# iamycy/golf

Hardware: AMD Instinct MI355X
Metric: audio samples/sec (24 kHz) GOLF-ss synth, batch=32x2 s, 4 batches in flight (higher is better)
Workload: dtype f32

## Files before the change

golf_amd/csrc/device_common.h:

```cpp
#pragma once
#include <hip/hip_runtime.h>

namespace golf {

struct BufRow {
    __amdgpu_buffer_rsrc_t rs;
    __device__ __forceinline__ BufRow(const float* p, int T)
        : rs(__builtin_amdgcn_make_buffer_rsrc((void*)p, 0, T * 4, 0x00020000)) {}
    __device__ __forceinline__ float ld(int t) const {
        return __builtin_bit_cast(float, __builtin_amdgcn_raw_buffer_load_b32(rs, t * 4, 0, 0));
    }
    __device__ __forceinline__ void st(int t, float v) const {
        __builtin_amdgcn_raw_buffer_store_b32(__builtin_bit_cast(unsigned, v), rs, t * 4, 0, 0);
    }
};

template <int W, int ROWS = 64>
struct Tile {
    static constexpr int LD = W + 1;
    static constexpr int SIZE = ROWS * LD;
    static constexpr int ITS = ROWS * W / 64;

    __device__ static __forceinline__ void rowcol(int it, int lq, int lr, int& row, int& col) {
        const int q = (it * 64) / W, r = (it * 64) % W;
        col = r + lr;
        row = q + lq;
        if (col >= W) { col -= W; row += 1; }
        if (col >= W) { col -= W; row += 1; }
    }
    template <int DIR = 1>
    __device__ static __forceinline__ void fetch(float (&r)[ITS], const BufRow& src, int tbase, int L, int lq,
                                                 int lr) {
#pragma unroll
        for (int it = 0; it < ITS; ++it) {
            int row, col;
            rowcol(it, lq, lr, row, col);
            r[it] = src.ld(tbase + row * L + DIR * col);
        }
    }
    template <int DIR = 1>
    __device__ static __forceinline__ void store(const float (&r)[ITS], const BufRow& dst, int tbase, int L, int lq,
                                                 int lr) {
#pragma unroll
        for (int it = 0; it < ITS; ++it) {
            int row, col;
            rowcol(it, lq, lr, row, col);
            dst.st(tbase + row * L + DIR * col, r[it]);
        }
    }
    __device__ static __forceinline__ void scatter(float* lds, const float (&r)[ITS], int lq, int lr) {
#pragma unroll
        for (int it = 0; it < ITS; ++it) {
            int row, col;
            rowcol(it, lq, lr, row, col);
            lds[row * LD + col] = r[it];
        }
    }
    __device__ static __forceinline__ void gather(float (&r)[ITS], const float* lds, int lq, int lr) {
#pragma unroll
        for (int it = 0; it < ITS; ++it) {
            int row, col;
            rowcol(it, lq, lr, row, col);
            r[it] = lds[row * LD + col];
        }
    }
    __device__ static __forceinline__ void rows_load(float (&x)[W], const float* lds, int row) {
#pragma unroll
        for (int s = 0; s < W; ++s) x[s] = lds[row * LD + s];
    }
    __device__ static __forceinline__ void rows_store(float* lds, const float (&x)[W], int row) {
#pragma unroll
        for (int s = 0; s < W; ++s) lds[row * LD + s] = x[s];
    }
};

#ifndef GOLF_PRIO_LIGHT
#define GOLF_PRIO_LIGHT 1
#endif
__device__ __forceinline__ void light_wave_priority() {
#if GOLF_PRIO_LIGHT > 0
    __builtin_amdgcn_s_setprio(GOLF_PRIO_LIGHT);
#endif
}

__device__ __forceinline__ void wave_lds_fence() {
    __builtin_amdgcn_fence(__ATOMIC_RELEASE, "wavefront", "local");
    __builtin_amdgcn_wave_barrier();
    __builtin_amdgcn_fence(__ATOMIC_ACQUIRE, "wavefront", "local");
}

__device__ __forceinline__ float lane_bcast(float v, int lane) {
    return __int_as_float(__builtin_amdgcn_readlane(__float_as_int(v), lane));
}
__device__ __forceinline__ float f4get(const float4& v, int k) {
    return k == 0 ? v.x : (k == 1 ? v.y : (k == 2 ? v.z : v.w));
}


constexpr int quad_tpl(int W, int NT) {
    for (int d = 1; d <= W; ++d)
        if (W % d == 0 && 4 * d >= NT) return d;
    return W;
}
template <int CTRL>
__device__ __forceinline__ float dppf(float v) {
    return __builtin_bit_cast(float, __builtin_amdgcn_update_dpp(0, __builtin_bit_cast(int, v), CTRL, 0xF, 0xF, false));
}
#define DPP_XOR1 0xB1
#define DPP_XOR2 0x4E
#define DPP_SHR1 0x90
#define DPP_SHL1 0xF9
#define DPP_BC0  0x00


}
```

golf_amd/csrc/lpc_ss.hip:

```cpp
#include "common.h"
#include "device_common.h"
#include "lpc_p1f.h"
#include <cstdlib>

namespace golf {

struct WNT { int W, NT; };
static const WNT kTable[] = {{8, 2},   {8, 4},   {8, 6},   {16, 8},  {16, 12}, {16, 14}, {24, 8},  {24, 12},
                             {24, 16}, {24, 20}, {24, 22}, {32, 16}, {32, 22}, {32, 26}, {32, 30}, {40, 22},
                             {40, 26}, {40, 32}, {40, 38}};

#ifndef GOLF_SS_SERIAL_MIN_BATCH
#define GOLF_SS_SERIAL_MIN_BATCH 2048
#endif

bool make_ss_plan(int B, int T, int F, int M, int hop, SsPlan* p, int mode) {
    p->W = 0;
    p->NT = 0;
    p->serial = mode == GOLF_SS_SERIAL || (mode != GOLF_SS_CHUNKED && B >= GOLF_SS_SERIAL_MIN_BATCH);
    if (F >= 2) {
        for (const WNT& e : kTable) {
            if (e.NT < M || hop % e.W != 0) continue;
            if (p->W == 0 || e.NT < p->NT || (e.NT == p->NT && e.W < p->W)) { p->W = e.W; p->NT = e.NT; }
        }
    }
    if (p->W == 0) { p->total = 256; return false; }
    const int W = p->W;
    int L;
    const int target = 240;
    if (hop >= target) {
        L = W;
        for (int cand = W; cand <= 256 && cand <= hop; cand += W)
            if (hop % cand == 0) L = cand;
    } else {
        L = hop * (target / hop);
    }
    p->L = L;
    p->NC = (int)ceil_div(T, L);
    p->NP = p->NC - 1;
    p->seg = L < hop ? L : hop;
    p->NSEG = (int)ceil_div(T, p->seg);
    size_t o = 0;
    if (p->serial) {
        p->off_phi = p->off_phiT = p->off_z = p->off_E = p->off_z2 = p->off_S = p->off_zadj = p->off_lam = 0;
        p->NG = p->GS = 0;
        p->off_mt = p->off_gv = p->off_pmax = 0;
        p->off_tier = p->off_S1 = p->off_status = p->off_phi64 = p->off_fixcnt = 0;
        p->off_m64 = p->off_v64 = p->off_g64 = 0;
        p->off_mtT = p->off_L1 = p->off_wadj = p->off_dadj = 0;
        p->off_gflag = 0;
        p->off_g = o;    o = align_up(o + sizeof(float) * (size_t)B * T, 256);
        p->off_pa = o;   o = align_up(o + sizeof(float) * (size_t)B * p->NSEG * 2 * W, 256);
        p->off_pg = o;   o = align_up(o + sizeof(float) * (size_t)B * p->NSEG * 2, 256);
        p->total = o;
        return true;
    }
    p->off_phi = o;  o = align_up(o + sizeof(float) * (size_t)B * (p->NP > 0 ? p->NP : 1) * p->NT * W, 256);
    p->off_phiT = o; o = align_up(o + sizeof(float) * (size_t)B * (p->NP > 0 ? p->NP : 1) * p->NT * W, 256);
    p->off_z = o;    o = align_up(o + sizeof(float) * (size_t)B * (p->NP > 0 ? p->NP : 1) * W, 256);
    p->off_E = o;    o = align_up(o + sizeof(float) * (size_t)B * (p->NP > 0 ? p->NP : 1) * W, 256);
    p->off_z2 = o;   o = align_up(o + sizeof(float) * (size_t)B * (p->NP > 0 ? p->NP : 1) * W, 256);
    p->off_S = o;    o = align_up(o + sizeof(float) * (size_t)B * p->NC * 64, 256);
    p->off_zadj = o; o = align_up(o + sizeof(float) * (size_t)B * p->NC * W, 256);
    p->off_lam = o;  o = align_up(o + sizeof(float) * (size_t)B * p->NC * 64, 256);
    p->off_g = o;    o = align_up(o + sizeof(float) * (size_t)B * T, 256);
    p->off_pa = o;   o = align_up(o + sizeof(float) * (size_t)B * p->NSEG * 2 * W, 256);
    p->off_pg = o;   o = align_up(o + sizeof(float) * (size_t)B * p->NSEG * 2, 256);
    p->off_pmax = o; o = align_up(o + sizeof(float) * (size_t)B * (p->NP > 0 ? p->NP : 1), 256);
    p->off_tier = o; o = align_up(o + sizeof(unsigned) * ((size_t)B * 2 + 2), 256);
    p->off_status = o; o = align_up(o + sizeof(unsigned) * 8, 256);
    p->off_fixcnt = o; o = align_up(o + sizeof(unsigned) * ((size_t)B * 5 + 1), 256);
    p->NG = 0;
    p->GS = 0;
    p->off_mt = p->off_gv = o;
    if (p->NP >= 48 && p->NT <= 24) {
        p->GS = 16;
        p->NG = (int)ceil_div(p->NP, p->GS);
        p->off_mt = o;   o = align_up(o + sizeof(float) * (size_t)B * p->NG * p->NT * W, 256);
        p->off_gv = o; o = align_up(o + sizeof(float) * (size_t)B * p->NG * 32 * 2, 256);
    }
    p->off_S1 = o;   o = align_up(o + sizeof(float) * (size_t)B * p->NC * 32, 256);
    p->off_mtT = o;  o = align_up(o + sizeof(float) * (size_t)B * (p->NG > 0 ? p->NG : 1) * p->NT * W, 256);
    p->off_L1 = o;   o = align_up(o + sizeof(float) * (size_t)B * (p->NC + 1) * 32, 256);
    p->off_wadj = o; o = align_up(o + sizeof(float) * (size_t)B * (p->NG > 0 ? p->NG : 1) * 32 * 2, 256);
    p->off_dadj = o; o = align_up(o + sizeof(float) * (size_t)B * p->NC * W, 256);
    p->off_phi64 = o; o = align_up(o + sizeof(double) * (size_t)B * (p->NP > 0 ? p->NP : 1) * p->NT * W, 256);
    p->off_m64 = o;  o = align_up(o + sizeof(double) * (size_t)B * (p->NG > 0 ? p->NG : 1) * p->NT * W, 256);
    p->off_v64 = o;  o = align_up(o + sizeof(double) * (size_t)B * (p->NG > 0 ? p->NG : 1) * 32, 256);
    p->off_g64 = o;  o = align_up(o + sizeof(double) * (size_t)B * (p->NG + 1) * 32, 256);
    p->off_gflag = o; o = align_up(o + sizeof(unsigned) * (size_t)B * (p->NG + 1), 256);
    p->total = o;
    return true;
}

static float phi_guard() {
    static const float v = [] { const char* e = getenv("GOLF_SS_PHI_GUARD"); return e ? (float)atof(e) : 30.f; }();
    return v;
}
static float phi_guard2() {
    static const float v = [] { const char* e = getenv("GOLF_SS_PHI_GUARD2"); return e ? (float)atof(e) : 8.f; }();
    return v;
}
static float group_log2_guard() {
    static const float v = [] { const char* e = getenv("GOLF_SS_GROUP_LOG2"); return e ? (float)atof(e) : 96.f; }();
    return v;
}
static int hot_all_16ths() {
    static const int v = [] { const char* e = getenv("GOLF_SS_HOT_ALL_16THS"); return e ? atoi(e) : 16; }();
    return v;
}
static int hot_count() {
    static const int v = [] { const char* e = getenv("GOLF_SS_HOT_COUNT"); return e ? atoi(e) : 160; }();
    return v;
}
static float phi_guard3() {
    static const float v = [] { const char* e = getenv("GOLF_SS_PHI_GUARD3"); return e ? (float)atof(e) : 256.f; }();
    return v;
}
static bool serial_strides_ok(int64_t s0, int64_t s1) { return s0 < (1 << 24) && s1 < (1 << 24); }
constexpr unsigned kTierHot = 2u, kTierPrecise = 3u;
constexpr unsigned kScanTwoLevel = 0x2C0DE001u, kScanFlat = 0x2C0DE002u;
__device__ __forceinline__ void record_scan_kind(const unsigned* tier, int B, unsigned kind) {
    if (tier) { unsigned* w = const_cast<unsigned*>(tier); w[2 * B] = kind; w[2 * B + 1] = 0u; }
}
__device__ __forceinline__ void check_scan_kind(const unsigned* tier, int B, unsigned kind) {
    if (tier && tier[2 * B] != kind) const_cast<unsigned*>(tier)[2 * B + 1] = 1u;
}
__device__ __forceinline__ bool tier3(const unsigned* __restrict__ tier, int b) {
    return tier != nullptr && __builtin_amdgcn_readfirstlane((int)tier[2 * b]) == (int)kTierPrecise;
}

template <int W, int NT, int MODE, bool LS = false>
__device__ __forceinline__ void fwdq_body(const float* __restrict__ ex, int64_t ex_stride,
                                          const float* __restrict__ gain, const float* __restrict__ a,
                                          const float* __restrict__ S, float* __restrict__ out, int64_t y_stride, int T,
                                          int F, int M, int hop, int L, int NCQ, int NCS,
                                          const float* __restrict__ zin, float* __restrict__ xt,
                                          float* __restrict__ yt, int b, int cg, int lane,
                                          const float* lst = nullptr, float* ldl = nullptr,
                                          unsigned* __restrict__ nonfinite = nullptr) {
    constexpr int TPL = quad_tpl(W, NT);
    constexpr bool WY = MODE == 1;
    static_assert(MODE >= 0 && MODE <= 3 && (MODE != 3 || LS), "MODE 3 exists only with LDS-resident start states");
    constexpr int R = 16;
    using TL = Tile<W, R>;
    const int lq = lane / W, lr = lane % W;
    const int row = lane >> 2, r = lane & 3;
    const int c0 = cg * R;
    const int c = c0 + row;
    const bool mine = c < NCQ;
    const BufRow xrow(ex + (size_t)b * ex_stride, T);
    const BufRow yrow(WY ? out + (size_t)b * y_stride : nullptr, WY ? T : 0);
    float w[TPL];
    if (MODE >= 1 && mine) {
        if constexpr (LS) {
#pragma unroll
            for (int k = 0; k < TPL; ++k) w[TPL - 1 - k] = lst[row * 32 + r * TPL + k];
        } else {
            const float* sp = S + ((size_t)b * NCS + c) * 64 + r * TPL;
#pragma unroll
            for (int k = 0; k < TPL; ++k) w[TPL - 1 - k] = sp[k];
        }
    } else {
#pragma unroll
        for (int k = 0; k < TPL; ++k) w[k] = 0.f;
    }
    float a0[TPL], dd[TPL];
#pragma unroll
    for (int k = 0; k < TPL; ++k) { a0[k] = 0.f; dd[k] = 0.f; }
    float g0 = 0.f, dg = 0.f;
    const float inv_hop = 1.0f / (float)hop;
    int fcur = -1;
    const int nblk = L / W;
    float nx[TL::ITS];
    bool bad = false;
    TL::fetch(nx, xrow, c0 * L, L, lq, lr);
    for (int blk = 0; blk < nblk; ++blk) {
        const int tw = c0 * L + blk * W;
        if (tw >= T) break;
        TL::scatter(xt, nx, lq, lr);
        wave_lds_fence();
        float xin[W];
        TL::rows_load(xin, xt, row);
        TL::fetch(nx, xrow, tw + W, L, lq, lr);
        const int t0 = c * L + blk * W;
        const bool act = mine && t0 < T;
        float keep[W / 4];
#pragma unroll
        for (int j = 0; j < W / 4; ++j) keep[j] = 0.f;
        if (act) {
            int f = t0 / hop;
            if (f > F - 2) f = F - 2;
            if (f != fcur) {
                fcur = f;
                const float* pa0 = a + ((size_t)b * F + f) * M;
                const float* pa1 = pa0 + M;
#pragma unroll
                for (int k = 0; k < TPL; ++k) {
                    const int i = r * TPL + k;
                    const float v0 = i < M ? pa0[i] : 0.f;
                    const float v1 = i < M ? pa1[i] : 0.f;
                    a0[k] = v0;
                    dd[k] = (v1 - v0) * inv_hop;
                }
                g0 = gain[(size_t)b * F + f];
                dg = (gain[(size_t)b * F + f + 1] - g0) * inv_hop;
            }
            const float n0 = (float)(t0 - f * hop);
#pragma unroll
            for (int s = 0; s < W; ++s) {
                const float n = n0 + (float)s;
                const float x = xin[s] * fmaf(n, dg, g0);
                float cf[TPL];
#pragma unroll
                for (int k = 0; k < TPL; ++k) cf[k] = fmaf(n, dd[k], a0[k]);
                float pa = 0.f, pb = 0.f;
#pragma unroll
                for (int k = TPL - 1; k >= 1; --k) {
                    const int slot = (s - 1 - k + 4 * TPL) % TPL;
                    if (k & 1) pa = fmaf(cf[k], w[slot], pa);
                    else       pb = fmaf(cf[k], w[slot], pb);
                }
                float part = fmaf(cf[0], w[(s - 1 + TPL) % TPL], pa + pb);
                part += dppf<DPP_XOR1>(part);
                part += dppf<DPP_XOR2>(part);
                const float y = x - part;
                const float oldest = w[s % TPL];
                const float inc = dppf<DPP_SHR1>(oldest);
                w[s % TPL] = r == 0 ? y : inc;
                if (WY) keep[s >> 2] = ((s & 3) == r) ? y : keep[s >> 2];
            }
        }
        if (WY) {
#pragma unroll
            for (int j = 0; j < W / 4; ++j) yt[row * TL::LD + 4 * j + r] = keep[j];
            wave_lds_fence();
            float o[TL::ITS];
            TL::gather(o, yt, lq, lr);
            TL::store(o, yrow, tw, L, lq, lr);
#pragma unroll
            for (int it = 0; it < TL::ITS; ++it) bad = bad || !(fabsf(o[it]) <= 3.4028235e38f);
        }
        wave_lds_fence();
    }
    if (WY && nonfinite && __builtin_amdgcn_ballot_w64(bad) != 0ull && lane == 0) atomicOr(nonfinite, 1u);
    if (!WY && mine) {
        float* zp = out + ((size_t)b * NCQ + c) * W;
#pragma unroll
        for (int k = 0; k < TPL; ++k) {
            const int i = r * TPL + k;
            if (i < W) {
                float v = i < M ? w[TPL - 1 - k] : 0.f;
                if (MODE == 2) v -= S[((size_t)b * NCS + c + 1) * 64 + i];
                if constexpr (MODE == 3) {
                    v -= lst[(row + 1) * 32 + i];
                    ldl[row * 32 + i] = v;
                    if (!out) continue;
                }
                if constexpr (MODE == 0) {
                    if (ldl) ldl[row * 32 + i] = v;
                }
                zp[i] = v;
            }
        }
    }
}

template <int W, int NT, int MODE>
__global__ __launch_bounds__(64) void lpc_fwdq_kernel(const float* __restrict__ ex, int64_t ex_stride,
                                                      const float* __restrict__ gain, const float* __restrict__ a,
                                                      const float* __restrict__ S, float* __restrict__ out,
                                                      int64_t y_stride, int T, int F, int M, int hop, int L, int NCQ,
                                                      int NCS, const float* __restrict__ zin,
                                                      const unsigned* __restrict__ tier = nullptr) {
    using TL = Tile<W, 16>;
    __shared__ float xt[TL::SIZE];
    __shared__ float yt[MODE == 1 ? TL::SIZE : 1];
    if (MODE == 2 && tier3(tier, blockIdx.y)) return;
    fwdq_body<W, NT, MODE>(ex, ex_stride, gain, a, S, out, y_stride, T, F, M, hop, L, NCQ, NCS, zin, xt, yt,
                           blockIdx.y, blockIdx.x, threadIdx.x);
}

template <int CTRL>
__device__ __forceinline__ float dpp_row(float v) {
    return __builtin_bit_cast(float, __builtin_amdgcn_update_dpp(0, __builtin_bit_cast(int, v), CTRL, 0xF, 0xF, true));
}
template <int W, int NT, int LPU, bool STATE = false>
__device__ __forceinline__ void serial_fwd_unit(int unit, float* __restrict__ xt, float* __restrict__ yt,
                                                const float* __restrict__ ex, int64_t ex_stride,
                                                const float* __restrict__ gain, const float* __restrict__ a,
                                                float* __restrict__ y, int64_t y_stride, int B, int T, int F, int M,
                                                int hop, float* state = nullptr) {
    static_assert(LPU == 4 || LPU == 8, "a quad or half a DPP row per utterance");
    constexpr int ROWS = 64 / LPU;
    constexpr int TPL = LPU == 4 ? quad_tpl(W, NT) : (NT + LPU - 1) / LPU;
    static_assert(W % LPU == 0 && W % TPL == 0, "the unrolled block is whole turns of the history ring and of the output slots");
    using TL = Tile<W, ROWS>;
    const int lane = threadIdx.x & 63;
    const int lq = lane / W, lr = lane % W;
    const int row = lane / LPU, r = lane % LPU;
    const int b0 = unit * ROWS;
    if (b0 >= B) return;
    const int nrow = B - b0 < ROWS ? B - b0 : ROWS;
    const int b = b0 + (row < nrow ? row : nrow - 1);
    const int xs = (int)ex_stride, ys = (int)y_stride;
    const BufRow xblk(ex + (size_t)b0 * ex_stride, nrow * xs);
    const BufRow yblk(y + (size_t)b0 * y_stride, nrow * ys);
    auto fetch = [&](float (&v)[TL::ITS], int t0) {
#pragma unroll
        for (int it = 0; it < TL::ITS; ++it) {
            int rw, col;
            TL::rowcol(it, lq, lr, rw, col);
            const int t = t0 + col;
            v[it] = xblk.ld((t < T && rw < nrow) ? rw * xs + t : -1);
        }
    };
    auto load_row = [&](float (&dst)[TPL], int f) {
        const float* pa = a + ((size_t)b * F + f) * M;
#pragma unroll
        for (int k = 0; k < TPL; ++k) {
            const int i = r * TPL + k;
            dst[k] = pa[i < M ? i : 0];
            if (i >= M) dst[k] = 0.f;
        }
    };
    const float inv_hop = 1.0f / (float)hop;
    float w[TPL], a0[TPL], a1[TPL], an[TPL], dd[TPL];
#pragma unroll
    for (int k = 0; k < TPL; ++k) w[k] = 0.f;
    if constexpr (STATE) {
#pragma unroll
        for (int k = 0; k < TPL; ++k) {
            const int i = r * TPL + k;
            w[TPL - 1 - k] = i < M ? state[(size_t)b * M + i] : 0.f;
        }
    }
    int f = 0, n0 = 0;
    load_row(a0, 0);
    load_row(a1, 1);
    load_row(an, F > 2 ? 2 : F - 1);
    const float* gb = gain + (size_t)b * F;
    float g0 = gb[0], g1 = gb[1], gn = gb[F > 2 ? 2 : F - 1];
    float dg = (g1 - g0) * inv_hop;
#pragma unroll
    for (int k = 0; k < TPL; ++k) dd[k] = (a1[k] - a0[k]) * inv_hop;
    float nx[TL::ITS];
    fetch(nx, 0);
    for (int t0 = 0; t0 < T; t0 += W) {
        TL::scatter(xt, nx, lq, lr);
        wave_lds_fence();
        float xin[W];
        TL::rows_load(xin, xt, row);
        fetch(nx, t0 + W);
        if (n0 == hop && f < F - 2) {
            ++f;
            n0 = 0;
#pragma unroll
            for (int k = 0; k < TPL; ++k) { a0[k] = a1[k]; a1[k] = an[k]; dd[k] = (a1[k] - a0[k]) * inv_hop; }
            g0 = g1; g1 = gn; dg = (g1 - g0) * inv_hop;
            const int fn = f + 2 < F ? f + 2 : F - 1;
            load_row(an, fn);
            gn = gb[fn];
        }
        float keep[W / LPU];
#pragma unroll
        for (int j = 0; j < W / LPU; ++j) keep[j] = 0.f;
        const float nb = (float)n0;
#pragma unroll
        for (int s = 0; s < W; ++s) {
            const float n = nb + (float)s;
            const float x = xin[s] * fmaf(n, dg, g0);
            float cf[TPL];
#pragma unroll
            for (int k = 0; k < TPL; ++k) cf[k] = fmaf(n, dd[k], a0[k]);
            float pa = 0.f, pb = 0.f;
#pragma unroll
            for (int k = TPL - 1; k >= 1; --k) {
                const int slot = (s - 1 - k + 4 * TPL) % TPL;
                if (k & 1) pa = fmaf(cf[k], w[slot], pa);
                else       pb = fmaf(cf[k], w[slot], pb);
            }
            float part = fmaf(cf[0], w[(s - 1 + TPL) % TPL], pa + pb);
            part += dppf<DPP_XOR1>(part);
            part += dppf<DPP_XOR2>(part);
            if (LPU == 8) part += dpp_row<0x141>(part);
            const float yv = x - part;
            const float oldest = w[s % TPL];
            const float inc = LPU == 4 ? dppf<DPP_SHR1>(oldest) : dpp_row<0x111>(oldest);
            w[s % TPL] = r == 0 ? yv : inc;
            keep[s / LPU] = ((s % LPU) == r) ? yv : keep[s / LPU];
        }
        n0 += W;
#pragma unroll
        for (int j = 0; j < W / LPU; ++j) yt[row * TL::LD + LPU * j + r] = keep[j];
        wave_lds_fence();
        float o[TL::ITS];
        TL::gather(o, yt, lq, lr);
// ... 1615 lines not shown
            FQM_STAMP(3);
            __builtin_amdgcn_fence(__ATOMIC_RELEASE, "workgroup");
            __builtin_amdgcn_s_waitcnt(0x0F70);
            if (lane == 0) __hip_atomic_store(fl + g, 1u, __ATOMIC_RELAXED, __HIP_MEMORY_SCOPE_AGENT);
        }
        FQM_STAMP(4);
        const int npred = g < NG ? g : NG;
        auto wait_and_stage = [&]() {
            for (unsigned it = 0u;; ++it) {
                bool ok = true;
                for (int l = lane; l < npred; l += 64)
                    ok = ok && __hip_atomic_load(fl + l, __ATOMIC_RELAXED, __HIP_MEMORY_SCOPE_AGENT) != 0u;
                if (__builtin_amdgcn_ballot_w64(!ok) == 0ull) break;
                __builtin_amdgcn_s_sleep(2);
                if (it > (1u << 17)) { timed_out(); break; }
            }
            FQM_STAMP(5);
            __builtin_amdgcn_fence(__ATOMIC_ACQUIRE, "workgroup");
            const float* vsrc = Vd + (size_t)b * NG * 32;
            float tmp[kMergedMaxGroups / 2];
#pragma unroll
            for (int u = 0; u < kMergedMaxGroups / 2; ++u) {
                const int e = lane + 64 * u;
                tmp[u] = e < npred * 32 ? __hip_atomic_load(vsrc + e, __ATOMIC_RELAXED, __HIP_MEMORY_SCOPE_AGENT) : 0.f;
            }
#pragma unroll
            for (int u = 0; u < kMergedMaxGroups / 2; ++u) vdl[lane + 64 * u] = tmp[u];
            wave_lds_fence();
        };
        group_prologue<W, NT, THIN, true, decltype(wait_and_stage), LM ? 2 : 0>(PhiT, MT, vdl, dl, st, b, g, NP, NG, lane, nullptr,
                                                                               wait_and_stage, mapl);
        for (int e = lane; e < (kGroup + 1) * 32; e += 64) st[e] += s1l[e];
    } else {
        for (unsigned it = 0u; __hip_atomic_load(ready + b, __ATOMIC_RELAXED, __HIP_MEMORY_SCOPE_AGENT) == 0u; ++it) {
            __builtin_amdgcn_s_sleep(8);
            if (it > (1u << 16)) { timed_out(); break; }
        }
        __builtin_amdgcn_fence(__ATOMIC_ACQUIRE, "agent");
        if (__hip_atomic_load(arrived + 2 * B + b, __ATOMIC_RELAXED, __HIP_MEMORY_SCOPE_AGENT) != 0u) {
            for (int e = lane; e < (kGroup + 1) * 32; e += 64)
                st[e] = c0 + e / 32 <= NP ? s1b[(size_t)c0 * 32 + e] : 0.f;
        } else {
            for (int e = lane; e < (kGroup + 1) * 32; e += 64) st[e] = 0.f;
            wave_lds_fence();
            const int c1 = c0 + kGroup < NP ? c0 + kGroup : NP;
            const int n = c1 > c0 ? c1 - c0 : 0;
            const int cs = c0 < NP ? c0 : (NP > 0 ? NP - 1 : 0);
            precise_scan_range<W, NT, float, float>(Phi64 + ((size_t)b * NP + cs) * NT * W, z + ((size_t)b * NP + cs) * W, W, st,
                                                    32, n, lane, G64 + ((size_t)b * (NG + 1) + g) * 32);
        }
    }
    if (lost)
        for (int e = lane; e < (kGroup + 1) * 32; e += 64) st[e] = __builtin_nanf("");
    wave_lds_fence();
    FQM_STAMP(6);
    fwdq_body<W, NT, 1, true>(ex, ex_stride, gain, a, nullptr, y, y_stride, T, F, M, hop, L, NC, 0, nullptr, xt, yt, b, g, lane,
                              st, dl, nonfinite);
    FQM_STAMP(7);
#undef FQM_STAMP
}

template <int W, int NT, int D, bool ACC>
__global__ __launch_bounds__(64) void lpc_p2_scan_kernel(const float* __restrict__ PhiT, const float* __restrict__ z,
                                                         float* __restrict__ S, int NC, int NP, int B,
                                                         const unsigned* __restrict__ tier,
                                                         const double* __restrict__ Phi64,
                                                         unsigned* __restrict__ nonfinite = nullptr) {
    const int i = threadIdx.x;
    if (!ACC && blockIdx.x == 0 && i == 0) {
        record_scan_kind(tier, B, kScanFlat);
        if (nonfinite) nonfinite[0] = 0u;
    }
    if ((int)blockIdx.x >= B) {
        const int bp = (int)blockIdx.x - B;
        if (tier3(tier, bp))
            precise_fwd_scan<W, NT>(Phi64 + (size_t)bp * NP * NT * W, z + (size_t)bp * NP * W, S + (size_t)bp * NC * 64, 64,
                                    NP, i);
        return;
    }
    const int b = blockIdx.x;
    if (tier3(tier, b)) return;
    const bool act = i < NT;
    const int ii = act ? i : 0;
    float* Sb = S + (size_t)b * NC * 64 + i;
    if (NP <= 0) { if (!ACC) Sb[0] = 0.f; return; }
    const float4* rows = reinterpret_cast<const float4*>(PhiT + ((size_t)b * NP * NT + ii) * W);
    const size_t cstride4 = (size_t)NT * W / 4;
    const float* zb = z + (size_t)b * NP * W + ii;
    float4 buf[D][W / 4];
    float zc[D];
#pragma unroll
    for (int u = 0; u < D; ++u) {
        const int cl = u < NP ? u : NP - 1;
#pragma unroll
        for (int k = 0; k < W / 4; ++k) buf[u][k] = rows[(size_t)cl * cstride4 + k];
        zc[u] = zb[(size_t)cl * W];
    }
    float s = 0.f;
#define GOLF_P2_STEP(u)                                                              \
    {                                                                                \
        float acc0 = zc[u], acc1 = 0.f, acc2 = 0.f, acc3 = 0.f;                      \
        _Pragma("unroll") for (int j = 0; j < NT; ++j) {                             \
            const float pj = f4get(buf[u][j / 4], j % 4);                            \
            const float sj = lane_bcast(s, j);                                       \
            if ((j & 3) == 0) acc0 = fmaf(pj, sj, acc0);                             \
            else if ((j & 3) == 1) acc1 = fmaf(pj, sj, acc1);                        \
            else if ((j & 3) == 2) acc2 = fmaf(pj, sj, acc2);                        \
            else acc3 = fmaf(pj, sj, acc3);                                          \
        }                                                                            \
        s = act ? (acc0 + acc1) + (acc2 + acc3) : 0.f;                               \
    }
    int c0 = 0;
    for (; c0 + D <= NP; c0 += D) {
#pragma unroll
        for (int u = 0; u < D; ++u) {
            const int c = c0 + u;
            if (ACC) Sb[(size_t)c * 64] += s; else Sb[(size_t)c * 64] = s;
            GOLF_P2_STEP(u)
            const int cn = c + D < NP ? c + D : NP - 1;
#pragma unroll
            for (int k = 0; k < W / 4; ++k) buf[u][k] = rows[(size_t)cn * cstride4 + k];
            zc[u] = zb[(size_t)cn * W];
        }
    }
#pragma unroll
    for (int u = 0; u < D; ++u) {
        const int c = c0 + u;
        if (c < NP) {
            if (ACC) Sb[(size_t)c * 64] += s; else Sb[(size_t)c * 64] = s;
            GOLF_P2_STEP(u)
        }
    }
#undef GOLF_P2_STEP
    if (ACC) Sb[(size_t)NP * 64] += s; else Sb[(size_t)NP * 64] = s;
}

template <int W, int NT, int MODE, bool LS = false>
__device__ __forceinline__ void adjq_body(const float* __restrict__ gy, int64_t gy_stride, const float* __restrict__ a,
                                          const float* __restrict__ lamEnd, float* __restrict__ out, int64_t g_stride,
                                          int T, int F, int M, int hop, int L, int NC, int NCQ,
                                          float* __restrict__ xt, float* __restrict__ yt, int b, int cg, int lane,
                                          const float* lst = nullptr, float* ldl = nullptr) {
    constexpr int TPL = quad_tpl(W, NT);
    constexpr int R = 16;
    using TL = Tile<W, R>;
    static_assert(MODE >= 0 && MODE <= 3 && (MODE != 3 || LS), "MODE 3 exists only with LDS-resident states");
    const int lq = lane / W, lr = lane % W;
    const int row = lane >> 2, r = lane & 3;
    const int c0 = cg * R;
    const int c = c0 + row;
    const bool mine = c < NCQ;
    const BufRow gyrow(gy + (size_t)b * gy_stride, T);
    const BufRow grow(MODE == 1 ? out + (size_t)b * g_stride : nullptr, MODE == 1 ? T : 0);
    float p[TPL];
    if (MODE >= 1 && mine) {
        if constexpr (LS) {
#pragma unroll
            for (int k = 0; k < TPL; ++k) p[k] = lst[(row + 1) * 32 + r * TPL + k];
        } else {
            const float* lp = lamEnd + ((size_t)b * NC + c) * 64 + r * TPL;
#pragma unroll
            for (int k = 0; k < TPL; ++k) p[k] = lp[k];
        }
    } else {
#pragma unroll
        for (int k = 0; k < TPL; ++k) p[k] = 0.f;
    }
    float a0[TPL], dd[TPL];
#pragma unroll
    for (int k = 0; k < TPL; ++k) { a0[k] = 0.f; dd[k] = 0.f; }
    const float inv_hop = 1.0f / (float)hop;
    int fcur = -1;
    const int nblk = L / W;
    int blk = nblk - 1;
    while (blk > 0 && c0 * L + blk * W >= T) --blk;
    float nx[TL::ITS];
    TL::fetch(nx, gyrow, c0 * L + blk * W, L, lq, lr);
    for (; blk >= 0; --blk) {
        const int tw = c0 * L + blk * W;
        TL::scatter(xt, nx, lq, lr);
        wave_lds_fence();
        float gin[W];
        TL::rows_load(gin, xt, row);
        TL::fetch(nx, gyrow, tw - W, L, lq, lr);
        const int t0 = c * L + blk * W;
        const bool act = mine && t0 < T;
        float keep[W / 4];
#pragma unroll
        for (int j = 0; j < W / 4; ++j) keep[j] = 0.f;
        if (act) {
            int f = t0 / hop;
            if (f > F - 2) f = F - 2;
            if (f != fcur) {
                fcur = f;
                const float* pa0 = a + ((size_t)b * F + f) * M;
                const float* pa1 = pa0 + M;
#pragma unroll
                for (int k = 0; k < TPL; ++k) {
                    const int i = r * TPL + k;
                    const float v0 = i < M ? pa0[i] : 0.f;
                    const float v1 = i < M ? pa1[i] : 0.f;
                    a0[k] = v0;
                    dd[k] = (v1 - v0) * inv_hop;
                }
            }
            const float n0 = (float)(t0 - f * hop);
#pragma unroll
            for (int s = W - 1; s >= 0; --s) {
                const int st = W - 1 - s;
                const float n = n0 + (float)s;
                const float head = p[st % TPL];
                const float g = dppf<DPP_BC0>(gin[s] + head);
                float inc = dppf<DPP_SHL1>(head);
                inc = r == 3 ? 0.f : inc;
#pragma unroll
                for (int k = 0; k < TPL - 1; ++k) {
                    const float cf = fmaf(n, dd[k], a0[k]);
                    p[(k + st + 1) % TPL] = fmaf(-cf, g, p[(k + st + 1) % TPL]);
                }
                const float cfl = fmaf(n, dd[TPL - 1], a0[TPL - 1]);
                p[st % TPL] = fmaf(-cfl, g, inc);
                if (MODE == 1) keep[s >> 2] = ((s & 3) == r) ? g : keep[s >> 2];
            }
        }
        if (MODE == 1) {
#pragma unroll
            for (int j = 0; j < W / 4; ++j) yt[row * TL::LD + 4 * j + r] = keep[j];
            wave_lds_fence();
            float o[TL::ITS];
            TL::gather(o, yt, lq, lr);
            TL::store(o, grow, tw, L, lq, lr);
        }
        wave_lds_fence();
    }
    if (MODE != 1 && mine) {
        float* zp = out + ((size_t)b * NC + c) * W;
#pragma unroll
        for (int k = 0; k < TPL; ++k) {
            const int i = r * TPL + k;
            if (i < W) {
                float v = i < NT ? p[k] : 0.f;
                if (MODE == 2) v = c >= 1 ? v - lamEnd[((size_t)b * NC + c - 1) * 64 + i] : 0.f;
                if constexpr (MODE == 3) v = c >= 1 ? v - lst[row * 32 + i] : 0.f;
                if (MODE != 2 && ldl) ldl[row * 32 + i] = v;
                zp[i] = v;
            }
        }
    }
}

template <int W, int NT, int MODE>
__global__ __launch_bounds__(64) void lpc_adjq_kernel(const float* __restrict__ gy, int64_t gy_stride,
                                                      const float* __restrict__ a, const float* __restrict__ lamEnd,
                                                      float* __restrict__ out, int64_t g_stride, int T, int F, int M,
                                                      int hop, int L, int NC, const unsigned* __restrict__ tier = nullptr) {
    using TL = Tile<W, 16>;
    __shared__ float xt[TL::SIZE];
    __shared__ float yt[MODE == 1 ? TL::SIZE : 1];
    if (MODE == 0 && blockIdx.x == 0 && blockIdx.y == 0 && threadIdx.x == 0) check_scan_kind(tier, (int)gridDim.y, kScanFlat);
    if (MODE == 2 && tier3(tier, blockIdx.y)) return;
    adjq_body<W, NT, MODE>(gy, gy_stride, a, lamEnd, out, g_stride, T, F, M, hop, L, NC, NC, xt, yt, blockIdx.y, blockIdx.x,
                           threadIdx.x);
}

template <int W, int NT>
__device__ __forceinline__ void adj_group_prologue(const float* __restrict__ Phi, const float* __restrict__ MTt,
                                                   const float* __restrict__ Wv, const float* __restrict__ x, int NC,
                                                   bool with_top, float* __restrict__ st, int b, int g, int NP, int NG,
                                                   int lane) {
    const bool act = lane < NT;
    const int ii = act ? lane : 0;
    const size_t cstride4 = (size_t)NT * W / 4;
    const int c0 = g * kGroup;
    const int gt = NG - 1;
    const int ct = c0 + kGroup - 1 < NP - 1 ? c0 + kGroup - 1 : NP - 1;
    constexpr int DC = kPrefetchMaps;
    const float4* rows = reinterpret_cast<const float4*>(Phi + ((size_t)b * NP * NT + ii) * W);
    const float* xb = x + (size_t)b * NC * W + ii;
    float4 pb[DC][W / 4];
    float xx[DC];
    auto fetchc = [&](int u, int c) {
        const int cl = c < 0 ? 0 : (c < NP ? c : NP - 1);
#pragma unroll
        for (int k = 0; k < W / 4; ++k) pb[u][k] = rows[(size_t)cl * cstride4 + k];
        xx[u] = xb[(size_t)cl * W];
    };
#pragma unroll
    for (int u = 0; u < DC; ++u) fetchc(u, ct - u);
    float t = (with_top && act) ? x[((size_t)b * NC + NP) * W + ii] : 0.f;
    if (g < gt) {
        constexpr int D = kPrefetchComposites;
        const float4* mrows = reinterpret_cast<const float4*>(MTt + ((size_t)b * NG * NT + ii) * W);
        const float* vb = Wv + (size_t)b * NG * 32 + ii;
        float4 mb[D][W / 4];
        float vv[D];
        auto fetch = [&](int u, int gg) {
            const int gl = gg > g ? gg : g + 1;
#pragma unroll
            for (int k = 0; k < W / 4; ++k) mb[u][k] = mrows[(size_t)gl * cstride4 + k];
            vv[u] = vb[(size_t)gl * 32];
        };
#pragma unroll
        for (int u = 0; u < D; ++u) fetch(u, gt - u);
        for (int gb = gt; gb > g; gb -= D) {
#pragma unroll
            for (int u = 0; u < D; ++u) {
                if (gb - u > g) {
                    t = matvec_step<W, NT>(mb[u], t, vv[u], act);
                    fetch(u, gb - u - D);
                }
            }
        }
    }
    for (int e = lane; e < (kGroup + 1) * 32; e += 64) st[e] = 0.f;
    wave_lds_fence();
    if (c0 <= NP - 1) {
#pragma unroll
        for (int k = 0; k < kGroup; ++k) {
            const int u = k % DC;
            const int c = ct - k;
            if (c >= c0) {
                if (lane < 32) st[(c - c0 + 1) * 32 + lane] = t;
                t = matvec_step<W, NT>(pb[u], t, xx[u], act);
                if (k + DC < kGroup) fetchc(u, c - DC);
            }
        }
        if (lane < 32) st[lane] = t;
    }
    wave_lds_fence();
}

template <int W, int NT, int MODE>
__global__ __launch_bounds__(64) void lpc_adjq2_kernel(const float* __restrict__ gy, int64_t gy_stride,
                                                       const float* __restrict__ a, float* __restrict__ out,
                                                       int64_t g_stride, int T, int F, int M, int hop, int L, int NC,
                                                       const float* __restrict__ Phi, const float* __restrict__ MTt,
                                                       const float* __restrict__ Wv, float* __restrict__ Wout,
                                                       const float* __restrict__ x, int NP, int NG,
                                                       float* __restrict__ L1, const unsigned* __restrict__ tier, int B,
                                                       const double* __restrict__ Phi64, const double* __restrict__ M64,
                                                       double* __restrict__ W64, double* __restrict__ GA64,
                                                       unsigned* __restrict__ arrived, const float* __restrict__ zq) {
    static_assert(MODE == 0 || MODE == 1 || MODE == 3, "local adjoints, final pass or refinement pass");
    using TL = Tile<W, 16>;
    __shared__ float xt[TL::SIZE];
    __shared__ float yt[MODE == 1 ? TL::SIZE : 1];
    __shared__ float st[(kGroup + 1) * 32];
    __shared__ float dl[kGroup * 32];
    if constexpr (MODE == 0) {
        if (blockIdx.x == 0 && blockIdx.y == 0 && threadIdx.x == 0) check_scan_kind(tier, B, kScanTwoLevel);
    }
    if constexpr (MODE == 3) {
        if ((int)blockIdx.y >= B) {
            const int w = ((int)blockIdx.y - B) * (int)gridDim.x + (int)blockIdx.x;
            const int nw = ((int)gridDim.y - B) * (int)gridDim.x;
            for (int job = w; job < B * NG; job += nw) {
                const int bp = job / NG, gj = job - bp * NG;
                if (!tier3(tier, bp)) continue;
                if (arrived[2 * B + bp] != 0u) {
                    if (gj == 0)
                        precise_adj_scan<W, NT>(Phi64 + (size_t)bp * NP * NT * W, x + (size_t)bp * NC * W,
                                                L1 + (size_t)bp * (NC + 1) * 32 + 32, 32, NP, threadIdx.x);
                } else {
                    precise_adj_group_job<W, NT>(Phi64, x, M64, W64, GA64, arrived, bp, gj, NP, NC, NG, threadIdx.x);
                }
            }
            return;
        }
    }
    const int b = blockIdx.y, g = blockIdx.x, lane = threadIdx.x;
    const int c0 = g * kGroup;
    const bool precise = tier3(tier, b);
    float* l1b = L1 + (size_t)b * (NC + 1) * 32;
    const bool act = lane < NT;
    const int ii = act ? lane : 0;
    if constexpr (MODE == 0) {
        for (int e = lane; e < kGroup * 32; e += 64) dl[e] = 0.f;
        wave_lds_fence();
        adjq_body<W, NT, 0>(gy, gy_stride, a, nullptr, out, 0, T, F, M, hop, L, NC, NC, xt, yt, b, g, lane, nullptr, dl);
        if (g >= NG || precise) return;
    } else if constexpr (MODE == 3) {
        if (precise) return;
        float4 mb[W / 4];
        float vv;
        {
            const float4* mrow = reinterpret_cast<const float4*>(MTt + (((size_t)b * NG + g) * NT + ii) * W);
#pragma unroll
// ... 1089 lines not shown
```

Baseline: 22.29 billion.

## Pack LPC recurrence into paired float2 FMAs with DPP-fused shift helpers

```diff
diff --git a/golf_amd/csrc/device_common.h b/golf_amd/csrc/device_common.h
--- a/golf_amd/csrc/device_common.h
+++ b/golf_amd/csrc/device_common.h
@@ -112,5 +112,20 @@
 #define DPP_SHL1 0xF9
 #define DPP_BC0  0x00
 
+typedef float qf2 __attribute__((ext_vector_type(2)));
+__device__ __forceinline__ float quad_shift_in(float leaving, float fresh) {
+    register unsigned long long first asm("vcc") = 0x1111111111111111ull;
+    asm("s_nop 1\n\tv_cndmask_b32_dpp %0, %0, %1, vcc quad_perm:[0,0,1,2] row_mask:0xf bank_mask:0xf"
+        : "+v"(leaving) : "v"(fresh), "s"(first));
+    return leaving;
+}
+__device__ __forceinline__ float quad_head_shift_out(float& head, float x) {
+    register unsigned long long last asm("vcc") = 0x8888888888888888ull;
+    float g;
+    asm("s_nop 1\n\tv_add_f32_dpp %0, %1, %2 quad_perm:[0,0,0,0] row_mask:0xf bank_mask:0xf\n\t"
+        "v_cndmask_b32_dpp %1, %1, %3, vcc quad_perm:[1,2,3,3] row_mask:0xf bank_mask:0xf"
+        : "=&v"(g), "+v"(head) : "v"(x), "v"(0.f), "s"(last));
+    return g;
+}
 
 }
diff --git a/golf_amd/csrc/lpc_ss.hip b/golf_amd/csrc/lpc_ss.hip
--- a/golf_amd/csrc/lpc_ss.hip
+++ b/golf_amd/csrc/lpc_ss.hip
@@ -151,24 +151,29 @@
     const bool mine = c < NCQ;
     const BufRow xrow(ex + (size_t)b * ex_stride, T);
     const BufRow yrow(WY ? out + (size_t)b * y_stride : nullptr, WY ? T : 0);
-    float w[TPL];
+    constexpr bool PK = TPL % 2 == 0;
+    constexpr int NPR = (TPL + 1) / 2;
+    constexpr bool WIN = WY && 4 * TPL == W;
+    qf2 wp[NPR];
+#define WSLOT(k) wp[(k) >> 1][(k) & 1]
+#pragma unroll
+    for (int p = 0; p < NPR; ++p) wp[p] = qf2{0.f, 0.f};
     if (MODE >= 1 && mine) {
         if constexpr (LS) {
 #pragma unroll
-            for (int k = 0; k < TPL; ++k) w[TPL - 1 - k] = lst[row * 32 + r * TPL + k];
+            for (int k = 0; k < TPL; ++k) WSLOT(TPL - 1 - k) = lst[row * 32 + r * TPL + k];
         } else {
             const float* sp = S + ((size_t)b * NCS + c) * 64 + r * TPL;
 #pragma unroll
-            for (int k = 0; k < TPL; ++k) w[TPL - 1 - k] = sp[k];
-        }
-    } else {
-#pragma unroll
-        for (int k = 0; k < TPL; ++k) w[k] = 0.f;
-    }
-    float a0[TPL], dd[TPL];
-#pragma unroll
-    for (int k = 0; k < TPL; ++k) { a0[k] = 0.f; dd[k] = 0.f; }
-    float g0 = 0.f, dg = 0.f;
+            for (int k = 0; k < TPL; ++k) WSLOT(TPL - 1 - k) = sp[k];
+        }
+    }
+    qf2 a0A[NPR], ddA[NPR], a0B[NPR], ddB[NPR];
+#pragma unroll
+    for (int q = 0; q < NPR; ++q) a0A[q] = ddA[q] = a0B[q] = ddB[q] = qf2{0.f, 0.f};
+    qf2 gdg = {0.f, 0.f};
+    qf2 qz = {0.f, 0.f};
+    asm volatile("" : "+v"(qz));
     const float inv_hop = 1.0f / (float)hop;
     int fcur = -1;
     const int nblk = L / W;
@@ -185,9 +190,9 @@
         TL::fetch(nx, xrow, tw + W, L, lq, lr);
         const int t0 = c * L + blk * W;
         const bool act = mine && t0 < T;
-        float keep[W / 4];
-#pragma unroll
-        for (int j = 0; j < W / 4; ++j) keep[j] = 0.f;
+        float keep[WIN ? 1 : W / 4];
+#pragma unroll
+        for (int j = 0; j < (WIN ? 1 : W / 4); ++j) keep[j] = 0.f;
         if (act) {
             int f = t0 / hop;
             if (f > F - 2) f = F - 2;
@@ -200,40 +205,81 @@
                     const int i = r * TPL + k;
                     const float v0 = i < M ? pa0[i] : 0.f;
                     const float v1 = i < M ? pa1[i] : 0.f;
-                    a0[k] = v0;
-                    dd[k] = (v1 - v0) * inv_hop;
+                    const float d = (v1 - v0) * inv_hop;
+                    if (PK) {
+                        a0A[k >> 1][(k & 1) ^ 1] = v0;
+                        ddA[k >> 1][(k & 1) ^ 1] = d;
+                        a0B[((k + TPL - 1) % TPL) >> 1][k & 1] = v0;
+                        ddB[((k + TPL - 1) % TPL) >> 1][k & 1] = d;
+                    } else {
+                        a0A[k >> 1][k & 1] = v0;
+                        ddA[k >> 1][k & 1] = d;
+                    }
                 }
-                g0 = gain[(size_t)b * F + f];
-                dg = (gain[(size_t)b * F + f + 1] - g0) * inv_hop;
+                const float g0 = gain[(size_t)b * F + f];
+                gdg = qf2{g0, (gain[(size_t)b * F + f + 1] - g0) * inv_hop};
             }
             const float n0 = (float)(t0 - f * hop);
+            qf2 nn = {0.f, 0.f}, gg = {0.f, 0.f};
 #pragma unroll
             for (int s = 0; s < W; ++s) {
-                const float n = n0 + (float)s;
-                const float x = xin[s] * fmaf(n, dg, g0);
-                float cf[TPL];
-#pragma unroll
-                for (int k = 0; k < TPL; ++k) cf[k] = fmaf(n, dd[k], a0[k]);
-                float pa = 0.f, pb = 0.f;
-#pragma unroll
-                for (int k = TPL - 1; k >= 1; --k) {
-                    const int slot = (s - 1 - k + 4 * TPL) % TPL;
-                    if (k & 1) pa = fmaf(cf[k], w[slot], pa);
-                    else       pb = fmaf(cf[k], w[slot], pb);
+                if ((s & 1) == 0) {
+                    nn = qf2{n0, n0} + qf2{(float)s, (float)(s + 1)};
+                    gg = __builtin_elementwise_fma(nn, gdg.yy, gdg.xx);
                 }
-                float part = fmaf(cf[0], w[(s - 1 + TPL) % TPL], pa + pb);
+                const int o = s % TPL;
+                float part;
+                if constexpr (!PK) {
+                    const float n = nn[s & 1];
+                    float cf[TPL];
+#pragma unroll
+                    for (int k = 0; k < TPL; ++k) cf[k] = fmaf(n, ddA[k >> 1][k & 1], a0A[k >> 1][k & 1]);
+                    float pa = 0.f, pb = 0.f;
+#pragma unroll
+                    for (int k = TPL - 1; k >= 1; --k) {
+                        const int slot = (s - 1 - k + 4 * TPL) % TPL;
+                        if (k & 1) pa = fmaf(cf[k], WSLOT(slot), pa);
+                        else       pb = fmaf(cf[k], WSLOT(slot), pb);
+                    }
+                    part = fmaf(cf[0], WSLOT((s - 1 + TPL) % TPL), pa + pb);
+                } else if ((s & 1) == 0) {
+                    qf2 cf[NPR];
+#pragma unroll
+                    for (int q = 0; q < NPR; ++q) cf[q] = __builtin_elementwise_fma(nn.xx, ddA[q], a0A[q]);
+                    qf2 acc = {0.f, 0.f};
+#pragma unroll
+                    for (int m = 0; m < TPL - 2; m += 2)
+                        acc = __builtin_elementwise_fma(cf[(TPL - 2 - m) / 2], wp[((o + m) % TPL) / 2], acc);
+                    const qf2 nw = wp[((o + TPL - 2) % TPL) / 2];
+                    const float pa = fmaf(cf[0].x, nw.x, acc.x);
+                    part = fmaf(cf[0].y, nw.y, pa + acc.y);
+                } else {
+                    qf2 cf[NPR];
+#pragma unroll
+                    for (int q = 0; q < NPR; ++q) cf[q] = __builtin_elementwise_fma(nn.yy, ddB[q], a0B[q]);
+                    const qf2 ow = wp[(o - 1) / 2];
+                    qz.y = fmaf(cf[NPR - 1].y, ow.y, 0.f);
+                    qf2 acc = qz;
+#pragma unroll
+                    for (int m = 1; m < TPL - 1; m += 2)
+                        acc = __builtin_elementwise_fma(cf[(TPL - 3 - m) / 2], wp[((o + m) % TPL) / 2], acc);
+                    part = fmaf(cf[NPR - 1].x, ow.x, acc.y + acc.x);
+                }
                 part += dppf<DPP_XOR1>(part);
                 part += dppf<DPP_XOR2>(part);
-                const float y = x - part;
-                const float oldest = w[s % TPL];
-                const float inc = dppf<DPP_SHR1>(oldest);
-                w[s % TPL] = r == 0 ? y : inc;
-                if (WY) keep[s >> 2] = ((s & 3) == r) ? y : keep[s >> 2];
+                const float y = fmaf(xin[s], gg[s & 1], -part);
+                WSLOT(o) = quad_shift_in(WSLOT(o), y);
+                if (WY && !WIN) keep[s >> 2] = ((s & 3) == r) ? y : keep[s >> 2];
             }
         }
         if (WY) {
-#pragma unroll
-            for (int j = 0; j < W / 4; ++j) yt[row * TL::LD + 4 * j + r] = keep[j];
+            if constexpr (WIN) {
+#pragma unroll
+                for (int j = 0; j < TPL; ++j) yt[row * TL::LD + (3 - r) * TPL + j] = act ? WSLOT(j) : 0.f;
+            } else {
+#pragma unroll
+                for (int j = 0; j < W / 4; ++j) yt[row * TL::LD + 4 * j + r] = keep[j];
+            }
             wave_lds_fence();
             float o[TL::ITS];
             TL::gather(o, yt, lq, lr);
@@ -243,6 +289,10 @@
         }
         wave_lds_fence();
     }
+    float w[TPL];
+#pragma unroll
+    for (int k = 0; k < TPL; ++k) w[k] = WSLOT(k);
+#undef WSLOT
     if (WY && nonfinite && __builtin_amdgcn_ballot_w64(bad) != 0ull && lane == 0) atomicOr(nonfinite, 1u);
     if (!WY && mine) {
         float* zp = out + ((size_t)b * NCQ + c) * W;
@@ -2164,23 +2214,25 @@
     const bool mine = c < NCQ;
     const BufRow gyrow(gy + (size_t)b * gy_stride, T);
     const BufRow grow(MODE == 1 ? out + (size_t)b * g_stride : nullptr, MODE == 1 ? T : 0);
-    float p[TPL];
+    constexpr bool PK = TPL % 2 == 0;
+    constexpr int NPR = (TPL + 1) / 2;
+    qf2 pp[NPR];
+#define PSLOT(k) pp[(k) >> 1][(k) & 1]
+#pragma unroll
+    for (int j = 0; j < NPR; ++j) pp[j] = qf2{0.f, 0.f};
     if (MODE >= 1 && mine) {
         if constexpr (LS) {
 #pragma unroll
-            for (int k = 0; k < TPL; ++k) p[k] = lst[(row + 1) * 32 + r * TPL + k];
+            for (int k = 0; k < TPL; ++k) PSLOT(k) = lst[(row + 1) * 32 + r * TPL + k];
         } else {
             const float* lp = lamEnd + ((size_t)b * NC + c) * 64 + r * TPL;
 #pragma unroll
-            for (int k = 0; k < TPL; ++k) p[k] = lp[k];
-        }
-    } else {
-#pragma unroll
-        for (int k = 0; k < TPL; ++k) p[k] = 0.f;
-    }
-    float a0[TPL], dd[TPL];
-#pragma unroll
-    for (int k = 0; k < TPL; ++k) { a0[k] = 0.f; dd[k] = 0.f; }
+            for (int k = 0; k < TPL; ++k) PSLOT(k) = lp[k];
+        }
+    }
+    qf2 a0A[NPR], ddA[NPR], a0B[NPR], ddB[NPR];
+#pragma unroll
+    for (int q = 0; q < NPR; ++q) a0A[q] = ddA[q] = a0B[q] = ddB[q] = qf2{0.f, 0.f};
     const float inv_hop = 1.0f / (float)hop;
     int fcur = -1;
     const int nblk = L / W;
@@ -2212,26 +2264,44 @@
                     const int i = r * TPL + k;
                     const float v0 = i < M ? pa0[i] : 0.f;
                     const float v1 = i < M ? pa1[i] : 0.f;
-                    a0[k] = v0;
-                    dd[k] = (v1 - v0) * inv_hop;
+                    const float d = (v1 - v0) * inv_hop;
+                    a0A[k >> 1][k & 1] = v0;
+                    ddA[k >> 1][k & 1] = d;
+                    if (PK) {
+                        a0B[((k + TPL - 1) % TPL) >> 1][(k + TPL - 1) & 1] = v0;
+                        ddB[((k + TPL - 1) % TPL) >> 1][(k + TPL - 1) & 1] = d;
+                    }
                 }
             }
             const float n0 = (float)(t0 - f * hop);
+            qf2 nn = {0.f, 0.f};
 #pragma unroll
             for (int s = W - 1; s >= 0; --s) {
                 const int st = W - 1 - s;
-                const float n = n0 + (float)s;
-                const float head = p[st % TPL];
-                const float g = dppf<DPP_BC0>(gin[s] + head);
-                float inc = dppf<DPP_SHL1>(head);
-                inc = r == 3 ? 0.f : inc;
-#pragma unroll
-                for (int k = 0; k < TPL - 1; ++k) {
-                    const float cf = fmaf(n, dd[k], a0[k]);
-                    p[(k + st + 1) % TPL] = fmaf(-cf, g, p[(k + st + 1) % TPL]);
+                if (s & 1) nn = qf2{n0, n0} + qf2{(float)(s - 1), (float)s};
+                float head = PSLOT(st % TPL);
+                const float g = quad_head_shift_out(head, gin[s]);
+                PSLOT(st % TPL) = head;
+                if constexpr (!PK) {
+                    const float n = nn[s & 1];
+#pragma unroll
+                    for (int k = 0; k < TPL; ++k) {
+                        const float cf = fmaf(n, ddA[k >> 1][k & 1], a0A[k >> 1][k & 1]);
+                        PSLOT((k + st + 1) % TPL) = fmaf(-cf, g, PSLOT((k + st + 1) % TPL));
+                    }
+                } else if (st & 1) {
+#pragma unroll
+                    for (int q = 0; q < NPR; ++q) {
+                        const qf2 cf = __builtin_elementwise_fma(nn.xx, ddA[q], a0A[q]);
+                        pp[((2 * q + st + 1) % TPL) / 2] = __builtin_elementwise_fma(-cf, qf2{g, g}, pp[((2 * q + st + 1) % TPL) / 2]);
+                    }
+                } else {
+#pragma unroll
+                    for (int q = 0; q < NPR; ++q) {
+                        const qf2 cf = __builtin_elementwise_fma(nn.yy, ddB[q], a0B[q]);
+                        pp[((2 * q + st + 2) % TPL) / 2] = __builtin_elementwise_fma(-cf, qf2{g, g}, pp[((2 * q + st + 2) % TPL) / 2]);
+                    }
                 }
-                const float cfl = fmaf(n, dd[TPL - 1], a0[TPL - 1]);
-                p[st % TPL] = fmaf(-cfl, g, inc);
                 if (MODE == 1) keep[s >> 2] = ((s & 3) == r) ? g : keep[s >> 2];
             }
         }
@@ -2245,6 +2315,10 @@
         }
         wave_lds_fence();
     }
+    float p[TPL];
+#pragma unroll
+    for (int k = 0; k < TPL; ++k) p[k] = PSLOT(k);
+#undef PSLOT
     if (MODE != 1 && mine) {
         float* zp = out + ((size_t)b * NC + c) * W;
 #pragma unroll
```

New measurement: 20.63 billion. 0.925x the previous value.
